# ysong1231/SimRank

Hardware: AMD Instinct MI355X
Metric: simrank_iterations_per_sec (higher is better)
Workload: dtype f32

## Files before the change

simrank_amd/csrc/api.hip:

```cpp
#include <algorithm>
#include <chrono>
#include <cstring>
#include <mutex>
#include <unordered_map>
#include <string>
#include <thread>
#include <vector>

#include "common.h"

namespace simrank {

static thread_local char g_err[512] = "";

void set_error(const char* fmt, ...) {
    va_list ap;
    va_start(ap, fmt);
    vsnprintf(g_err, sizeof(g_err), fmt, ap);
    va_end(ap);
}

Tuning& tuning() {
    static Tuning t;
    return t;
// ... 884 lines not shown
    } else if (!strcmp(key, "fuse_sym")) {
        SR_REQUIRE(value >= -1 && value <= 1, "fuse_sym must be -1 (automatic), 0 or 1");
        t.fuse_sym = value;
    } else if (!strcmp(key, "fuse_steps")) {
        SR_REQUIRE(value >= -1 && value <= (1 << 20), "fuse_steps must be >= 0, or -1 (by the operand's size)");
        t.fuse_steps = value;
    } else if (!strcmp(key, "fuse_dens")) {
        SR_REQUIRE(value >= 0 && value <= (1 << 20), "fuse_dens must be >= 0");
        t.fuse_dens = value;
    } else if (!strcmp(key, "dense_cols")) {
        SR_REQUIRE(value >= 1 && value <= (1 << 20), "dense_cols must be >= 1");
        t.dense_cols = value;
    } else if (!strcmp(key, "restrict_support")) {
        SR_REQUIRE(value >= -1 && value <= 1, "restrict_support must be -1 (automatic), 0 or 1");
        t.restrict_support = value;
    } else {
        SR_REQUIRE(false, "unknown tuning key '%s'", key);
    }
    return SIMRANK_OK;
}

int simrank_get_tuning(const char* key, int64_t* value) {
    SR_REQUIRE(key && value, "NULL argument");
    const Tuning t = tuning_snapshot();
    if (!strcmp(key, "panel")) *value = t.panel;
    else if (!strcmp(key, "xcd_map")) *value = t.xcd_map;
    else if (!strcmp(key, "stream_nt")) *value = t.stream_nt;
    else if (!strcmp(key, "tile")) *value = t.tile;
    else if (!strcmp(key, "triangle")) *value = t.triangle;
    else if (!strcmp(key, "huge")) *value = t.huge;
// ... 15 lines not shown
    else if (!strcmp(key, "ev_tri")) *value = t.ev_tri;
    else if (!strcmp(key, "fuse_rows")) *value = t.fuse_rows;
    else if (!strcmp(key, "fuse_wgs")) *value = t.fuse_wgs;
    else if (!strcmp(key, "fuse_max_rows")) *value = t.fuse_max_rows;
    else if (!strcmp(key, "fuse_order")) *value = t.fuse_order;
    else if (!strcmp(key, "fuse_store")) *value = t.fuse_store;
    else if (!strcmp(key, "fuse_meta_nt")) *value = t.fuse_meta_nt;
    else if (!strcmp(key, "sym_desc")) *value = t.sym_desc;
    else if (!strcmp(key, "ids16")) *value = t.ids16;
    else if (!strcmp(key, "lean")) *value = t.lean;
    else if (!strcmp(key, "addr32")) *value = t.addr32;
    else if (!strcmp(key, "probe_flags")) *value = t.probe_flags;
    else if (!strcmp(key, "dense_terms")) *value = t.dense_terms;
    else if (!strcmp(key, "probe_mask")) *value = t.probe_mask;
    else if (!strcmp(key, "restrict_support")) *value = t.restrict_support;
    else SR_REQUIRE(false, "unknown tuning key '%s'", key);
    return SIMRANK_OK;
}

int simrank_graph_get(const simrank_graph* g, const char* key, int64_t* value) {
    SR_REQUIRE(g && key && value, "NULL argument");
    if (!strcmp(key, "fused_ids16")) *value = g->fused ? g->fused->ids16 : -1;
    else if (!strcmp(key, "gather_ids16")) *value = (g->col16 && g->tun.ids16) ? 1 : 0;
    else SR_REQUIRE(false, "unknown graph key '%s'", key);
    return SIMRANK_OK;
}

}
```

simrank_amd/csrc/common.h:

```cpp
#pragma once
#include <hip/hip_runtime.h>

#include <cstdarg>
#include <atomic>
#include <cstdint>
#include <cstdio>
#include <cstdlib>
#include <cstring>
#include <functional>
#include <vector>

#include "simrank_hip.h"

namespace simrank {

void set_error(const char* fmt, ...);

#define SR_HIP(call)                                                                   \
    do {                                                                               \
        hipError_t e_ = (call);                                                        \
        if (e_ != hipSuccess) {                                                        \
            ::simrank::set_error("%s failed: %s (%s:%d)", #call, hipGetErrorString(e_), \
                                 __FILE__, __LINE__);                                  \
            return SIMRANK_ERR_HIP;                                                    \
// ... 31 lines not shown
    int64_t fuse_min = 0;
    int64_t fuse_pays = -1;
    int64_t fuse_steps = -1;
    int64_t fuse_dens = 0;
    int64_t fuse_unit = 48;
    int64_t fuse_rows = 8192;
    int64_t fuse_store = 1;
    int64_t fuse_meta_nt = 0;
    int64_t fuse_order = 0;
    int64_t fuse_max_rows = 1 << 20;
    int64_t fuse_cap = 40000;
    int64_t fuse_wgs = 4;
    int64_t fuse_shards = 1;
    int64_t fuse_group = 3;
    int64_t fuse_sym = -1;
    int64_t dense_lazy = 0;
    int64_t dense_sym = -1;
    int64_t restrict_support = -1;
};
inline int32_t restrict_choice(const Tuning& t, int64_t live, int64_t total) {
    return t.restrict_support < 0 ? (2 * live < total ? 1 : 0) : int32_t(t.restrict_support != 0);
}
Tuning& tuning();
Tuning tuning_snapshot();


#ifdef SIMRANK_HOST_ONLY
inline hipError_t plan_alloc(void** p, size_t bytes) {
    *p = malloc(bytes ? bytes : 1);
    return *p ? hipSuccess : hipErrorOutOfMemory;
// ... 25 lines not shown
int rows_to_host(const void* S, int64_t rows_pad, int64_t n, const int32_t* inv_dev, const int32_t* rows, int32_t n_rows,
                 float* dst, int64_t ld, int elem, float scale, hipStream_t stream);
inline hipError_t pool_hip_alloc(void** p, size_t bytes) {
    const int rc = pool_alloc(p, bytes);
    return rc == SIMRANK_OK ? hipSuccess : (rc == SIMRANK_ERR_ALLOC ? hipErrorOutOfMemory : hipErrorUnknown);
}

int identity_leg1_blocked(const simrank_graph* g, float* Tt, int64_t t_rows_pad, void* stream);
int identity_leg1_blocked_h16(const simrank_graph* g, uint16_t* Tt, int64_t t_rows_pad, float scale, void* stream);

struct PlanPrep {
    std::vector<int32_t> ord, inv;
    std::vector<int32_t> rp, cl;
    std::vector<float> rs;
    bool asym = false;
};
struct BiPlanPrep {
    std::vector<int32_t> rowptr21, col21;
    std::vector<int32_t> ord[2], inv[2];
    std::vector<int32_t> rp[2], cl[2];
    std::vector<float> rs[2];
    bool asym = false;
};
int plan_prepare(int64_t n, int64_t nnz, const int32_t* rowptr, const int32_t* col, const float* rowscale,
                 const simrank_plan_options* opt, PlanPrep* out);
int shard_prepare(int64_t n, int64_t nnz, const int32_t* rowptr, const int32_t* col, const float* rowscale,
                  const float* apriori, int64_t ld_apriori, bool reorder, int32_t deal, PlanPrep* out, bool allow_asym = false);
int shard_biplan_prepare(int64_t n1, int64_t n2, int64_t nnz, const int32_t* rowptr12, const int32_t* col12,
                         const float* rowscale1, const float* rowscale2, const simrank_biplan_options* opt, int32_t deal1,
                         int32_t deal2, BiPlanPrep* out, bool allow_asym = false);
bool prior_symmetric(const float* a, int64_t ld, int64_t n);
// ... 45 lines not shown
    int64_t n_quads = 0;
    int64_t n_steps = 0;
    int64_t nnz_covered = 0;
    int64_t r_nnz = 0;
    int32_t* units = nullptr;
    int32_t n_pslots = 0, n_cslots = 0;
    float* partials = nullptr;
    int32_t* tickets = nullptr;
    int32_t cap_panels = 0;
    uint16_t* dcols16 = nullptr;
    int32_t* dcols32 = nullptr;
    uint4* abits = nullptr;
    int2* gmeta = nullptr;
    uint16_t* sids16 = nullptr;
    int32_t* sids32 = nullptr;
};

#ifdef SIMRANK_EXPERIMENT_FUSED2
struct simrank_fused2_plan {
    int32_t n_items = 0;
    int32_t n_blocks = 0;
    int32_t ids16 = 0;
    int32_t cap_panels = 0;
    int64_t n_quads = 0, n_steps = 0, nnz_covered = 0, r_nnz = 0;
    int32_t* items = nullptr;
    int32_t n_pslots = 0, n_cslots = 0;
    float* partials = nullptr;
    int32_t* tickets = nullptr;
    uint32_t* heads = nullptr;
    uint16_t* dcols16 = nullptr;
    int32_t* dcols32 = nullptr;
    uint4* abits = nullptr;
    int2* gmeta = nullptr;
    uint16_t* sids16 = nullptr;
    int32_t* sids32 = nullptr;
};
#endif

namespace simrank {
constexpr int kFB = 128;
constexpr int kSub = 4;
void free_fused_plan(simrank_fused_plan* p);
int build_fused_plan(simrank_graph* g, const int32_t* rowptr, const int32_t* col, const float* rowscale);
int launch_fused_trans(const simrank_graph* g, const float* X, int64_t x_rows_pad, int64_t L, float* Y,
                       int64_t y_rows_pad, hipStream_t st);
bool fused_sym_applies(const simrank_graph* g, int64_t x_rows_pad, int64_t L, int64_t y_rows_pad);
int launch_fused_sym(const simrank_graph* g, const float* X, int64_t x_rows_pad, int64_t L, float* Y, int64_t y_rows_pad,
                     float coef, float lbd, double eps, const uint8_t* ev, const float* ap, const float* prev,
                     unsigned long long* n_changed, int32_t set_diag, int32_t count_any, hipStream_t st);
bool fused_rowmajor_fits(const simrank_graph* g, const float* X, int64_t ldx, int64_t L, const float* Y, int64_t t_block,
                         int64_t t_pad);
int launch_fused_trans_rowmajor(const simrank_graph* g, const float* X, int64_t ldx, int64_t L, float* Y, int64_t t_block,
                                int64_t t_pad, hipStream_t st);
#ifdef SIMRANK_EXPERIMENT_FUSED2
void free_fused2_plan(simrank_fused2_plan* p);
int build_fused2_plan(simrank_graph* g, const int32_t* rowptr, const int32_t* col, const float* rowscale);
int launch_fused2_trans(const simrank_graph* g, const float* X, int64_t x_rows_pad, int64_t L, float* Y,
                        int64_t y_rows_pad, hipStream_t st);
#endif
struct DenseUse {
// ... 40 lines not shown
```

simrank_amd/csrc/fused.hip:

```cpp
#include <algorithm>
#include <cstring>
#include <numeric>
#include <vector>

#include <cstdlib>

#include <mutex>
#include <thread>

#include "common.h"
#include "fused_dev.h"

namespace simrank {

constexpr int kTS = 132;
#ifndef SIMRANK_KMINUNITS
#define SIMRANK_KMINUNITS 64
#endif
#ifndef SIMRANK_KGROUPENTRIES
#define SIMRANK_KGROUPENTRIES 6144
#endif
#ifndef SIMRANK_KMAXREM
#define SIMRANK_KMAXREM 256
#endif
// ... 23 lines not shown
    int32_t* tickets;
    int32_t n_pslots, n_cslots;
    const uint16_t* dcols16;
    const int32_t* dcols32;
    const uint4* abits;
    const int2* gmeta;
    const uint16_t* sids16;
    const int32_t* sids32;
    float coef, lbd;
    double eps;
    const uint8_t* ev;
    const float* ap;
    const float* prev;
    unsigned long long* n_changed;
    int32_t set_diag, count_any;
};

#ifndef SIMRANK_HOST_ONLY
#if defined(__HIP_DEVICE_COMPILE__) && !defined(__gfx942__) && !defined(__gfx950__)
#error "fused.hip: the sc1 hand-off between the units of a split block is written for gfx942 / gfx950"
#endif
#ifdef SIMRANK_FUSED_STAMPS
constexpr int kFstCap = 1 << 15;
__device__ unsigned long long g_fst[kFstCap * 8];
__device__ unsigned int g_fst_base;
__device__ __forceinline__ unsigned long long fst_now() {
    unsigned long long t;
    __builtin_amdgcn_sched_barrier(0);
    asm volatile("s_memtime %0\n\ts_waitcnt lgkmcnt(0)" : "=s"(t) :: "memory");
    __builtin_amdgcn_sched_barrier(0);
// ... 32 lines not shown
    const int32_t* un = p.units + size_t(unit) * 32;
    FST(0);
#ifdef SIMRANK_FUSED_STAMPS
    if (threadIdx.x == 0 && blockIdx.x - g_fst_base < unsigned(kFstCap)) {
        const unsigned xcc = __builtin_amdgcn_s_getreg((4 - 1) << 11 | 0 << 6 | 20);
        const unsigned hw = __builtin_amdgcn_s_getreg((16 - 1) << 11 | 0 << 6 | 4);
        g_fst[size_t(blockIdx.x - g_fst_base) * 8 + 5] = (unsigned long long)xcc << 32 | hw;
        g_fst[size_t(blockIdx.x - g_fst_base) * 8 + 6] = (unsigned long long)panel << 32 | unit;
    }
#endif
    const int b0 = un[0];
    const int64_t c0 = int64_t(panel) * 32;
    const int n_sub_all = un[8];
    const int n_sub_sym = SYM ? min(n_sub_all, int((c0 + 31) >> 7) - b0 + 1) : n_sub_all;
    if (SYM && n_sub_sym <= 0) return;
    const int g = lane >> 3, q = lane & 7, gbase = lane & ~7;
    const uint32_t qoff = uint32_t(q) * 16u;

    const float* xbase = p.X + int64_t(panel) * p.x_panel_stride;
    const __amdgpu_buffer_rsrc_t srd = __builtin_amdgcn_make_buffer_rsrc(
        const_cast<float*>(xbase), 0, p.x_bytes - (p.x_pitch == 128u ? 0 : panel * 128), 0x00020000);
    const uint32_t pitch = p.x_pitch;
    const int sent = p.x_sentinel;

    const int quad0 = un[1];
    const int nq = (p.probe & 4) ? 0 : un[2];
    const int unit_k = un[3], unit_nb = un[4], pslot = un[5], cslot = un[6];
    const bool has_set = !(p.probe & 4) && un[7] != 0;
    const int n_sub = n_sub_sym;
    const int per = (nq + 3) >> 2;
// ... 832 lines not shown
            std::fwrite(sids.data(), sizeof(int32_t), sids.size(), f);
            std::fwrite(dcols.data(), sizeof(int32_t), dcols.size(), f);
            std::fclose(f);
        }
    }
    simrank_fused_plan* pl = new simrank_fused_plan;
    pl->n_units = (int32_t)(units.size() / 32);
    pl->n_blocks = (int32_t)nblk;
    pl->n_pslots = n_pslots;
    pl->n_cslots = n_cslots;
    pl->n_quads = blk_quad0[size_t(nblk)];
    pl->n_steps = steps_total;
    pl->nnz_covered = covered;
    pl->r_nnz = r_nnz;
    pl->ids16 = ids16 ? 1 : 0;
    dcols.resize(dcols.size() + 64, 0);
    abits.resize(abits.size() + 64 * 4, 0u);
    int rc = upload_vec(&pl->units, units);
    if (!rc) {
        if (ids16) {
            std::vector<uint16_t> d16(dcols.begin(), dcols.end());
            rc = upload_vec(&pl->dcols16, d16);
        } else {
            rc = upload_vec(&pl->dcols32, dcols);
        }
    }
    if (!rc) rc = upload_vec(reinterpret_cast<uint32_t**>(&pl->abits), abits);
    if (!rc) rc = upload_vec(reinterpret_cast<int32_t**>(&pl->gmeta), blk_gmeta);
    if (!rc) {
        if (ids16) {
// ... 73 lines not shown
        if (pl->ids16)
            hipLaunchKernelGGL((fused_trans_kernel<true, true>), dim3((unsigned)grid), dim3(256), lds_pad, st, a);
        else
            hipLaunchKernelGGL((fused_trans_kernel<false, true>), dim3((unsigned)grid), dim3(256), lds_pad, st, a);
    } else if (pl->ids16) {
        hipLaunchKernelGGL((fused_trans_kernel<true, false>), dim3((unsigned)grid), dim3(256), lds_pad, st, a);
    } else {
        hipLaunchKernelGGL((fused_trans_kernel<false, false>), dim3((unsigned)grid), dim3(256), lds_pad, st, a);
    }
#endif
    SR_HIP(hipGetLastError());
    return SIMRANK_OK;
}

int launch_fused_trans(const simrank_graph* g, const float* X, int64_t x_rows_pad, int64_t L, float* Y,
                       int64_t y_rows_pad, hipStream_t st) {
    SR_REQUIRE(g->fused, "graph has no fused plan");
    SR_REQUIRE(aligned16(X) && aligned16(Y), "fused leg needs 16-byte aligned operands");
    SR_REQUIRE(x_rows_pad >= g->n_cols && (x_rows_pad + 1) * 128 < (int64_t(1) << 31) && x_rows_pad < (int64_t(1) << 24) - 1,
               "fused leg: operand of %lld rows per panel", (long long)x_rows_pad);
    FusedArgs a{};
    a.X = X; a.Y = Y;
    a.x_rows_pad = x_rows_pad; a.y_rows_pad = y_rows_pad;
    a.L = L;
    a.x_panel_stride = x_rows_pad * 32;
    a.x_pitch = 128;
    a.x_bytes = int32_t(x_rows_pad * 128);
    a.x_sentinel = (int32_t)x_rows_pad;
    return launch_fused(g, a, st);
}

bool fused_sym_applies(const simrank_graph* g, int64_t x_rows_pad, int64_t L, int64_t y_rows_pad) {
    const simrank_fused_plan* pl = g->fused;
    if (!pl || !g->tun.fuse || g->tun.fuse_sym == 0 || g->tun.dense_terms != 3) return false;
    if (L != g->n_rows || g->n_cols > g->tun.fuse_max_rows) return false;
    if ((x_rows_pad + 1) * 128 >= (int64_t(1) << 31) || (y_rows_pad + 1) * 128 >= (int64_t(1) << 31) ||
        x_rows_pad >= (int64_t(1) << 24) - 1 || y_rows_pad >= (int64_t(1) << 24) - 1)
        return false;
    if (g->tun.fuse_sym < 0) return 2 * pl->nnz_covered >= g->nnz;
    return true;
}

int launch_fused_sym(const simrank_graph* g, const float* X, int64_t x_rows_pad, int64_t L, float* Y, int64_t y_rows_pad,
                     float coef, float lbd, double eps, const uint8_t* ev, const float* ap, const float* prev,
// ... 72 lines not shown
```

simrank_amd/csrc/plan.hip:

```cpp
#include <algorithm>
#include <chrono>
#include <cstdlib>
#include <cstring>
#include <numeric>
#include <vector>

#include "loop.h"
#include "side.h"

struct simrank_plan {
    simrank::side_t s;
    unsigned long long* counters = nullptr;
    unsigned long long* host_counters[2] = {nullptr, nullptr};
    hipEvent_t counted[2] = {nullptr, nullptr};
    hipStream_t stream = nullptr;
    int32_t asym = 0;
    int32_t updates = 0;
    int32_t identity_leg1 = 1;
    int32_t at_identity = 0;
    std::vector<hipEvent_t> ev_pool;
    std::vector<hipEvent_t> ev_used;
    bool timing = false;
};

// ... 103 lines not shown
    }
    if (p->s.half && !p->s.g->fused) {
        set_error("storage_fp16 needs the one-launch plan (tuning fuse = 1) and a graph that has one");
        return fail(SIMRANK_ERR_INVALID);
    }
    auto counters = [&]() -> int {
        SIDE_HIP(pool_hip_alloc((void**)&p->counters, sizeof(unsigned long long) * SIMRANK_CHANGED_SLOTS));
        for (int i = 0; i < 2; ++i) {
            SIDE_HIP(hipHostMalloc((void**)&p->host_counters[i], sizeof(unsigned long long) * SIMRANK_CHANGED_SLOTS, hipHostMallocPortable));
            SIDE_HIP(hipEventCreateWithFlags(&p->counted[i], hipEventDisableTiming));
        }
        return SIMRANK_OK;
    };
    rc = counters();
    if (!rc) rc = side_alloc(a, pp.ord, pp.inv, p->stream);
    if (rc) return fail(rc);
    lap("matrices allocated, orders uploaded, stream drained");
    if (opt->evidence) rc = side_restrict(a, p->stream);
    if (!rc && opt->apriori) rc = side_prior(a, opt->apriori, opt->ld_apriori, p->stream);
    if (rc) return fail(rc);
    lap("live segments, prior");
    rc = simrank_plan_reset(p);
    if (rc) return fail(rc);
    lap("reset queued");
    *out = p;
    return SIMRANK_OK;
}

int simrank_plan_reset(simrank_plan* p) {
    SR_REQUIRE(p, "plan is NULL");
// ... 149 lines not shown
```

simrank_amd/csrc/planprep.hip:

```cpp
#include <algorithm>
#include <atomic>
#include <cmath>
#include <numeric>
#include <thread>

#include "common.h"

namespace simrank {

static int check_csr(int64_t n_rows, int64_t n_cols, int64_t nnz, const int32_t* rowptr, const int32_t* col) {
    SR_REQUIRE(rowptr[0] == 0 && rowptr[n_rows] == nnz, "rowptr does not span [0, nnz]");
    for (int64_t a = 0; a < n_rows; ++a)
        SR_REQUIRE(rowptr[a + 1] >= rowptr[a] && rowptr[a + 1] <= nnz, "rowptr not monotone at row %lld", (long long)a);
    for (int64_t j = 0; j < nnz; ++j) SR_REQUIRE(col[j] >= 0 && col[j] < n_cols, "column index %d out of range", col[j]);
    return SIMRANK_OK;
}

static int check_prior(const float* a, int64_t ld, int64_t n, int which, bool half, bool* asym = nullptr) {
    if (!a) return SIMRANK_OK;
    SR_REQUIRE(ld >= n, "prior %d: ld %lld < n", which, (long long)ld);
    for (int64_t i = 0; i < n; ++i)
        for (int64_t j = i; j < n; ++j) {
            const float v = a[i * ld + j];
            if (j > i && !(v == a[j * ld + i])) {
// ... 61 lines not shown
    }
    SR_REQUIRE(dup_row.load() < 0, "duplicate entry in row %d%s", ord[(size_t)dup_row.load()], what);
    return SIMRANK_OK;
}

static void length_order(int64_t n, const int32_t* rowptr, bool reorder, std::vector<int32_t>& ord, std::vector<int32_t>& inv) {
    ord.resize((size_t)n);
    inv.resize((size_t)n);
    std::iota(ord.begin(), ord.end(), 0);
    if (reorder)
        std::stable_sort(ord.begin(), ord.end(),
                         [rowptr](int32_t x, int32_t y) { return rowptr[x + 1] - rowptr[x] < rowptr[y + 1] - rowptr[y]; });
    for (int64_t r = 0; r < n; ++r) inv[(size_t)ord[(size_t)r]] = (int32_t)r;
}

static void deal_order(int64_t n, int32_t deal, std::vector<int32_t>& ord, std::vector<int32_t>& inv) {
    if (deal <= 1 || n % (32 * int64_t(deal))) return;
    const int64_t unit = n % (128 * int64_t(deal)) == 0 ? 128 : 32, per = n / (unit * deal);
    std::vector<int32_t> dealt((size_t)n);
    for (int64_t b = 0; b < per; ++b)
        for (int64_t w = 0; w < deal; ++w)
            for (int64_t i = 0; i < unit; ++i)
                dealt[(size_t)((w * per + b) * unit + i)] = ord[(size_t)((b * deal + w) * unit + i)];
    ord.swap(dealt);
    for (int64_t r = 0; r < n; ++r) inv[(size_t)ord[(size_t)r]] = (int32_t)r;
}

int plan_prepare(int64_t n, int64_t nnz, const int32_t* rowptr, const int32_t* col, const float* rowscale,
                 const simrank_plan_options* opt, PlanPrep* out) {
    SR_REQUIRE(opt && rowptr && rowscale && (col || nnz == 0) && n > 0 && nnz >= 0 && out, "bad plan arguments");
    SR_REQUIRE(n < (int64_t(1) << 24) - 16, "a plan holds at most 2^24 nodes");
    SR_REQUIRE(opt->dense_terms == 0 || opt->dense_terms == 1 || opt->dense_terms == 3, "dense_terms must be 0, 1 or 3");
    int rc = check_csr(n, n, nnz, rowptr, col);
    out->asym = false;
    if (!rc) rc = check_prior(opt->apriori, opt->ld_apriori, n, 1, opt->storage_fp16 != 0, &out->asym);
    if (rc) return rc;
    length_order(n, rowptr, opt->reorder != 0, out->ord, out->inv);
    return renamed(n, rowptr, col, rowscale, out->ord, out->inv, nnz, "", out->rp, out->cl, out->rs);
}

int shard_prepare(int64_t n, int64_t nnz, const int32_t* rowptr, const int32_t* col, const float* rowscale,
                  const float* apriori, int64_t ld_apriori, bool reorder, int32_t deal, PlanPrep* out, bool allow_asym) {
    SR_REQUIRE(rowptr && rowscale && (col || nnz == 0) && n > 0 && nnz >= 0 && out, "bad plan arguments");
    SR_REQUIRE(n < (int64_t(1) << 24) - 16, "a plan holds at most 2^24 nodes");
    int rc = check_csr(n, n, nnz, rowptr, col);
    out->asym = false;
    if (!rc) rc = check_prior(apriori, ld_apriori, n, 1, false, allow_asym ? &out->asym : nullptr);
    if (rc) return rc;
    length_order(n, rowptr, reorder, out->ord, out->inv);
    if (reorder) deal_order(n, deal, out->ord, out->inv);
    return renamed(n, rowptr, col, rowscale, out->ord, out->inv, nnz, "", out->rp, out->cl, out->rs);
}

// ... 75 lines not shown
```

simrank_amd/csrc/side.h:

```cpp
#pragma once
#include <cstring>
#include <vector>

#include "common.h"

namespace simrank {

constexpr float kHalfScale = 16384.0f;

#define SIDE_HIP(call)                                                                            \
    do {                                                                                          \
        hipError_t e_ = (call);                                                                   \
        if (e_ != hipSuccess) {                                                                   \
            set_error("%s failed: %s (%s:%d)", #call, hipGetErrorString(e_), __FILE__, __LINE__); \
            (void)hipGetLastError();                                                              \
            return e_ == hipErrorOutOfMemory ? SIMRANK_ERR_ALLOC : SIMRANK_ERR_HIP;               \
        }                                                                                         \
    } while (0)

struct side_t {
    int64_t n = 0, k = 0, rows_pad = 0, k_rows_pad = 0;
    size_t mat_bytes = 0, t_bytes = 0;
    simrank_graph* g = nullptr;
    float* S[2] = {nullptr, nullptr};
    float* Tt = nullptr;
    uint8_t* ev = nullptr;
    float* prior = nullptr;
    int32_t* inv = nullptr;
    int32_t* ord_dev = nullptr;
    std::vector<int32_t> ord;
    float coef = 0.8f, lbd = 0.f;
    int32_t restrict_support = 0;
    int32_t half = 0;
    int cur = 0;
};

inline size_t side_f32_bytes(const side_t& a) { return size_t((a.n + 31) / 32) * size_t(a.rows_pad) * 32 * sizeof(float); }

inline void side_shape(side_t& a, int64_t n, int64_t k, bool half) {
    a.n = n;
    a.k = k;
    a.half = half ? 1 : 0;
    a.rows_pad = (n + 7) / 8 * 8 + 8;
    a.k_rows_pad = (k + 7) / 8 * 8 + 8;
    const size_t panels = half ? size_t((n + 63) / 64) : size_t((n + 31) / 32);
    a.mat_bytes = panels * size_t(a.rows_pad) * 128;
    a.t_bytes = panels * size_t(a.k_rows_pad) * 128;
}

// ... 5 lines not shown
    SIDE_HIP(hipMemcpyAsync(a.inv, inv.data(), ids, hipMemcpyHostToDevice, st));
    a.ord = ord;
    SIDE_HIP(pool_hip_alloc((void**)&a.ord_dev, ids));
    SIDE_HIP(hipMemcpyAsync(a.ord_dev, a.ord.data(), ids, hipMemcpyHostToDevice, st));
    SIDE_HIP(hipStreamSynchronize(st));
    return SIMRANK_OK;
}

inline void side_trim(side_t& a) {
    (void)pool_free(a.S[0]); (void)pool_free(a.S[1]); (void)pool_free(a.Tt); (void)pool_free(a.prior);
    a.S[0] = a.S[1] = a.Tt = a.prior = nullptr;
}

inline void side_free(side_t& a) {
    side_trim(a);
    (void)pool_free(a.ev); (void)pool_free(a.inv); (void)pool_free(a.ord_dev);
    simrank_graph_destroy(a.g);
}

inline int side_reset(side_t& a, hipStream_t st) {
    a.cur = 0;
    if (a.half) return simrank_fill_identity_blocked_h16(a.S[0], a.n, a.n, a.rows_pad, 0, kHalfScale, st);
    return simrank_fill_identity_blocked(a.S[0], a.n, a.n, a.rows_pad, 0, st);
}

inline int side_evidence_alloc(side_t& a, int fill, hipStream_t st) {
    const size_t ev_bytes = size_t((a.n + 31) / 32) * size_t(a.rows_pad) * 32;
    hipError_t e = pool_hip_alloc((void**)&a.ev, ev_bytes);
    if (e == hipSuccess) e = hipMemsetAsync(a.ev, fill, ev_bytes, st);
    if (e != hipSuccess) {
        set_error("evidence counts: %s", hipGetErrorString(e));
// ... 24 lines not shown
        rc = simrank_permute_layout(tmp, n, 0, a.prior, 32, a.rows_pad, n, n, a.ord_dev, a.ord_dev, 4, st);
        e = hipStreamSynchronize(st);
    }
    (void)pool_free(tmp);
    if (e != hipSuccess) {
        set_error("plan prior upload: %s", hipGetErrorString(e));
        return SIMRANK_ERR_HIP;
    }
    return rc;
}

template <class Stamp>
int side_leg_pair(side_t& a, const side_t& o, bool from_identity, bool asym, double eps, int32_t exact_count,
                  unsigned long long* counters, unsigned long long* host_slot, hipStream_t st, Stamp&& stamp) {
    const int nx = a.cur ^ 1;
    int rc = stamp();
    if (rc) return rc;
    rc = from_identity ? (a.half ? identity_leg1_blocked_h16(a.g, reinterpret_cast<uint16_t*>(a.Tt), a.k_rows_pad, kHalfScale, st)
                                 : identity_leg1_blocked(a.g, a.Tt, a.k_rows_pad, st))
         : a.half ? simrank_spmm_blocked_h16(a.g, o.S[o.cur], o.rows_pad, a.k, a.Tt, a.k_rows_pad, 1, nullptr, 0, kHalfScale, st)
                  : simrank_spmm_blocked(a.g, o.S[o.cur], o.rows_pad, a.k, a.Tt, a.k_rows_pad, 1, nullptr, st);
    if (!rc) rc = stamp();
    if (rc) return rc;
    simrank_epilogue ep{};
    ep.coef = a.coef;
    ep.lbd = a.lbd;
    ep.evidence = a.ev;
    ep.ld_evidence = 32;
    ep.apriori = a.prior;
    ep.ld_apriori = 32;
    ep.previous = a.S[a.cur];
    ep.ld_previous = 32;
    ep.eps = eps;
    ep.n_changed = counters;
    ep.diag_col0 = 0;
    ep.set_diag = 1;
    ep.symmetric = 1;
    ep.restrict_support = a.restrict_support;
    ep.count_any = exact_count ? 0 : 1;
    if (asym) {
        ep.symmetric = 0;
        ep.restrict_support = 0;
        rc = simrank_spmm_blocked(a.g, a.Tt, a.k_rows_pad, a.n, a.S[nx], a.rows_pad, 1, nullptr, st);
        if (!rc) rc = simrank_epilogue_apply_blocked(a.S[nx], a.S[nx], a.n, a.n, a.rows_pad, &ep, st);
    } else {
        rc = a.half ? simrank_spmm_blocked_h16(a.g, a.Tt, a.k_rows_pad, a.n, a.S[nx], a.rows_pad, 0, &ep, a.rows_pad, kHalfScale, st)
                    : simrank_spmm_blocked(a.g, a.Tt, a.k_rows_pad, a.n, a.S[nx], a.rows_pad, 0, &ep, st);
    }
    if (!rc) rc = stamp();
    if (rc) return rc;
    SR_HIP(hipMemcpyAsync(host_slot, counters, sizeof(unsigned long long) * SIMRANK_CHANGED_SLOTS, hipMemcpyDeviceToHost, st));
    return SIMRANK_OK;
}

// ... 74 lines not shown
        const int64_t node = a.ord[(size_t)r];
        std::memcpy(idx_host + node * k, idx_s.data() + r * k, size_t(k) * sizeof(int32_t));
        std::memcpy(val_host + node * k, val_s.data() + r * k, size_t(k) * sizeof(float));
    }
    return SIMRANK_OK;
}

inline int side_get(const side_t& a, const char* key, int64_t* value) {
    if (!strcmp(key, "restrict_support")) *value = a.restrict_support;
    else if (!strcmp(key, "iterate")) *value = (int64_t)(uintptr_t)a.S[a.cur];
    else if (!strcmp(key, "iterate_layout")) *value = a.half ? 2 : 0;
    else if (!strcmp(key, "iterate_stride")) *value = a.rows_pad;
    else if (!strcmp(key, "iterate_rows") || !strcmp(key, "iterate_col_hi")) *value = a.n;
    else if (!strcmp(key, "iterate_col_lo")) *value = 0;
    else if (!strcmp(key, "ids")) *value = (int64_t)(uintptr_t)a.ord_dev;
    else SR_REQUIRE(false, "unknown plan key '%s'", key);
    return SIMRANK_OK;
}

}
```

simrank_amd/csrc/spmm.hip:

```cpp
#include <algorithm>
#include <type_traits>

#include <mutex>

#include "common.h"

namespace simrank {

__device__ __forceinline__ int64_t imin(int64_t a, int64_t b) { return a < b ? a : b; }

__device__ __forceinline__ int64_t elem_at(int64_t r, int64_t c, int64_t ld, int64_t rows_pad) {
    return rows_pad ? ((c >> 5) * rows_pad + r) * 32 + (c & 31) : r * ld + c;
}

struct SpmmArgs {
    const int32_t* rowptr;
    const int32_t* col;
    const uint16_t* col16;
    int32_t blocked;
    int64_t x_rows_pad, y_rows_pad;
    int64_t x_span_bytes;
    int32_t x_sentinel;
    int32_t addr32;
    int32_t sh_rank, sh_mb;
// ... 1772 lines not shown
    *total = n_rows * ((n_cols + 31) / 32);
    return SIMRANK_OK;
}

int simrank_fill_identity(float* S, int64_t n_rows, int64_t n_cols, int64_t ld, int64_t col0,
                          void* stream) {
    SR_REQUIRE(S && n_rows > 0 && n_cols > 0 && ld >= n_cols, "bad identity block");
    const int64_t total = n_rows * n_cols;
    const int grid = (int)std::min<int64_t>((total + 255) / 256, 256 * 16);
    hipLaunchKernelGGL(fill_identity_kernel, dim3(grid), dim3(256), 0, as_stream(stream), S,
                       n_rows, n_cols, ld, col0);
    SR_HIP(hipGetLastError());
    return SIMRANK_OK;
}

static int spmm_impl(const simrank_graph* g, const float* X, int64_t ldx, int64_t n_cols_x,
                     float* Y, int64_t ldy, int32_t transpose_out, int64_t t_block, int64_t t_pad,
                     const simrank_epilogue* ep, void* stream, bool blocked, int64_t x_rows_pad,
                     int64_t y_rows_pad) {
    SR_REQUIRE(t_pad >= 0 && t_pad < 4096, "t_pad out of range");
    SR_REQUIRE(g && X && Y, "NULL argument");
    const Tuning& T = g->tun;
    SR_REQUIRE(!(transpose_out && ep), "an epilogue needs transpose_out = 0");
    SpmmArgs a{};
    a.blocked = blocked ? 1 : 0;
    a.x_rows_pad = x_rows_pad;
    a.y_rows_pad = y_rows_pad;
    a.rowptr = g->rowptr;
    a.col = g->col;
    a.col16 = T.ids16 ? g->col16 : nullptr;
    a.rowscale = g->rowscale;
    a.huge_len = (int32_t)std::max<int64_t>(kHeavy, T.huge);
    a.has_huge = g->max_row_nnz >= a.huge_len ? 1 : 0;
    a.X = X;
// ... 27 lines not shown
        a.ld_prev = ep->ld_previous;
        a.eps = ep->eps;
        a.n_changed = ep->n_changed;
        a.diag_col0 = ep->diag_col0;
        a.set_diag = ep->set_diag;
        a.restrict_support = ep->restrict_support;
        a.count_any = ep->count_any;
        if (blocked) a.ld_ev = a.ld_ap = a.ld_prev = 32;
        SR_REQUIRE(!a.ev || a.ld_ev >= n_cols_x || blocked, "evidence ld too small");
        SR_REQUIRE(!a.ap || a.ld_ap >= n_cols_x || blocked, "apriori ld too small");
        SR_REQUIRE(!a.prev || ((a.ld_prev >= n_cols_x || blocked) && a.n_changed),
                   "previous needs ld >= columns and a counter");
        if (a.ev) vec_ok = vec_ok && (reinterpret_cast<uintptr_t>(a.ev) % 4 == 0) && a.ld_ev % 4 == 0;
        if (a.ap) vec_ok = vec_ok && aligned16(a.ap) && a.ld_ap % 4 == 0;
        if (a.prev) vec_ok = vec_ok && aligned16(a.prev) && a.ld_prev % 4 == 0;
        if (a.prev) SR_HIP(hipMemsetAsync(a.n_changed, 0, sizeof(unsigned long long) * SIMRANK_CHANGED_SLOTS, st));
    }
    int64_t panel = T.panel;
    if (panel == 0) panel = transpose_out ? 32 : 64;
    int64_t tile = T.tile;
    if (tile == 0) tile = 32;
    a.nt = (int32_t)T.stream_nt;
    const bool want_sym = ep && ep->symmetric && T.triangle && vec_ok && !transpose_out &&
                          n_cols_x == g->n_rows && ep->diag_col0 == 0 && g->n_rows >= 64;
    if (blocked && transpose_out && g->fused && T.fuse && vec_ok && T.dense_terms == 3 && g->n_cols <= T.fuse_max_rows &&
        (x_rows_pad + 1) * 128 < (int64_t(1) << 31)) {
#ifdef SIMRANK_EXPERIMENT_FUSED2
        if (T.fuse == 2 && g->fused2 && (g->fused2->n_pslots == 0 || (n_cols_x + 31) / 32 <= g->fused2->cap_panels))
            return launch_fused2_trans(g, X, x_rows_pad, n_cols_x, Y, y_rows_pad, st);
#endif
        return launch_fused_trans(g, X, x_rows_pad, n_cols_x, Y, y_rows_pad, st);
    }
    if (!blocked && transpose_out && g->fused && T.fuse && T.fuse_shards && vec_ok && T.dense_terms == 3 &&
        g->n_cols <= T.fuse_max_rows) {
        const int64_t tb = a.tstride ? g->n_rows : t_block, tp = a.tstride ? a.tstride - g->n_rows : t_pad;
        if (fused_rowmajor_fits(g, X, ldx, n_cols_x, Y, tb, tp))
            return launch_fused_trans_rowmajor(g, X, ldx, n_cols_x, Y, tb, tp, st);
    }
    if (blocked && want_sym && !transpose_out && ep && (!ep->restrict_support || T.fuse_sym > 0) &&
        fused_sym_applies(g, x_rows_pad, n_cols_x, y_rows_pad))
        return launch_fused_sym(g, X, x_rows_pad, n_cols_x, Y, y_rows_pad, a.coef, a.lbd, a.eps, a.ev, a.ap, a.prev, a.n_changed,
                                a.set_diag, a.count_any, st);
    const simrank_dense_plan* dp = (vec_ok && T.dense_min > 0 && tile == 32) ? g->dense : nullptr;
    if (dp && want_sym) {
        const int64_t mode = T.dense_sym;
        if (mode == 0 || (mode < 0 && 2 * dp->nnz_covered < g->nnz)) dp = nullptr;
    }
    if (dp) {
        DenseUse use;
        const int rc = launch_dense_tiles(g, X, blocked ? -x_rows_pad : ldx, n_cols_x, want_sym, st, &use);
        if (rc) return rc;
        a.dpart = use.part;
        a.ldp = use.ldp;
        a.dslab0 = use.block_slab0;
        a.dnslab = use.block_nslab;
        a.rowptr = dp->r_rowptr;
        a.col = dp->r_col;
        a.col16 = T.ids16 ? dp->r_col16 : nullptr;
        a.has_huge = dp->r_max_row >= a.huge_len ? 1 : 0;
    }
    if (T.balance) {
        const int32_t* tr0 = dp ? dp->r_tile_row0 : g->tile_row0;
// ... 141 lines not shown
    SR_REQUIRE(n_cols_x > 0 && ldx >= n_cols_x, "X: %lld columns, ld %lld", (long long)n_cols_x,
               (long long)ldx);
    SR_REQUIRE(transpose_out || ldy >= n_cols_x, "Y: ld %lld < %lld columns", (long long)ldy,
               (long long)n_cols_x);
    return spmm_impl(g, X, ldx, n_cols_x, Y, ldy, transpose_out, t_block, t_pad, ep, stream, false, 0, 0);
}

int simrank_spmm_blocked(const simrank_graph* g, const float* X, int64_t x_rows_pad, int64_t n_cols_x,
                         float* Y, int64_t y_rows_pad, int32_t transpose_out,
                         const simrank_epilogue* ep, void* stream) {
    SR_REQUIRE(g && n_cols_x > 0, "bad arguments");
    SR_REQUIRE(x_rows_pad >= g->n_cols && y_rows_pad >= (transpose_out ? n_cols_x : g->n_rows),
               "padded row counts %lld / %lld too small", (long long)x_rows_pad, (long long)y_rows_pad);
    return spmm_impl(g, X, 32, n_cols_x, Y, 32, transpose_out, 0, 0, ep, stream, true, x_rows_pad, y_rows_pad);
}

static int epilogue_apply_impl(const float* Q, int64_t ldq, float* Y, int64_t ldy, int64_t n_rows,
                               int64_t n_cols, const simrank_epilogue* ep, void* stream, int64_t rows_pad) {
    SR_REQUIRE(Q && Y && ep, "NULL argument");
    SR_REQUIRE(n_rows > 0 && n_cols > 0 && (rows_pad ? rows_pad >= n_rows : (ldq >= n_cols && ldy >= n_cols)),
               "bad block shape");
    SpmmArgs a{};
    a.y_rows_pad = rows_pad;
    a.has_ep = 1;
    a.coef = ep->coef;
    a.lbd = ep->lbd;
    a.ev = ep->evidence;
    a.ld_ev = ep->ld_evidence;
    a.ap = ep->apriori;
    a.ld_ap = ep->ld_apriori;
// ... 300 lines not shown
```

Baseline: 134.7.

## Skip leg-1 fused work units whose output the triangular second leg never reads

Builds a per-panel first-referenced-block table on the host and passes it to the fused transposed SpMM kernel. Work units whose last block falls before the first block the triangular symmetric second leg will read exit early. A refined node ordering (by length, then first reference) is added to concentrate skippable work. A dry-run of the spmm dispatcher checks that the second leg really is triangular before skipping is enabled. The cost is extra host preprocessing, a device table, and reliance on the triangle path only reading the upper part.

```diff
diff --git a/simrank_amd/csrc/api.hip b/simrank_amd/csrc/api.hip
--- a/simrank_amd/csrc/api.hip
+++ b/simrank_amd/csrc/api.hip
@@ -922,6 +922,11 @@
     } else if (!strcmp(key, "restrict_support")) {
         SR_REQUIRE(value >= -1 && value <= 1, "restrict_support must be -1 (automatic), 0 or 1");
         t.restrict_support = value;
+    } else if (!strcmp(key, "leg1_skip")) {
+        t.leg1_skip = value ? 1 : 0;
+    } else if (!strcmp(key, "leg1_order")) {
+        SR_REQUIRE(value >= -1 && value <= 1, "leg1_order must be -1 (by the graph's size), 0 or 1");
+        t.leg1_order = value;
     } else {
         SR_REQUIRE(false, "unknown tuning key '%s'", key);
     }
@@ -967,6 +972,8 @@
     else if (!strcmp(key, "dense_terms")) *value = t.dense_terms;
     else if (!strcmp(key, "probe_mask")) *value = t.probe_mask;
     else if (!strcmp(key, "restrict_support")) *value = t.restrict_support;
+    else if (!strcmp(key, "leg1_skip")) *value = t.leg1_skip;
+    else if (!strcmp(key, "leg1_order")) *value = t.leg1_order;
     else SR_REQUIRE(false, "unknown tuning key '%s'", key);
     return SIMRANK_OK;
 }
diff --git a/simrank_amd/csrc/common.h b/simrank_amd/csrc/common.h
--- a/simrank_amd/csrc/common.h
+++ b/simrank_amd/csrc/common.h
@@ -69,6 +69,8 @@
     int64_t fuse_shards = 1;
     int64_t fuse_group = 3;
     int64_t fuse_sym = -1;
+    int64_t leg1_skip = 1;
+    int64_t leg1_order = -1;
     int64_t dense_lazy = 0;
     int64_t dense_sym = -1;
     int64_t restrict_support = -1;
@@ -124,7 +126,10 @@
     std::vector<int32_t> rp, cl;
     std::vector<float> rs;
     bool asym = false;
-};
+    std::vector<int32_t> first_block;
+};
+constexpr int32_t kLeg1Never = 0x7FFFFFFF;
+void first_block_table(int64_t n, const int32_t* rp, const int32_t* cl, std::vector<int32_t>& first_block);
 struct BiPlanPrep {
     std::vector<int32_t> rowptr21, col21;
     std::vector<int32_t> ord[2], inv[2];
@@ -200,6 +205,7 @@
     int2* gmeta = nullptr;
     uint16_t* sids16 = nullptr;
     int32_t* sids32 = nullptr;
+    std::vector<int32_t> unit_last;
 };
 
 #ifdef SIMRANK_EXPERIMENT_FUSED2
@@ -229,7 +235,12 @@
 void free_fused_plan(simrank_fused_plan* p);
 int build_fused_plan(simrank_graph* g, const int32_t* rowptr, const int32_t* col, const float* rowscale);
 int launch_fused_trans(const simrank_graph* g, const float* X, int64_t x_rows_pad, int64_t L, float* Y,
-                       int64_t y_rows_pad, hipStream_t st);
+                       int64_t y_rows_pad, hipStream_t st, const int32_t* first_block = nullptr);
+void fused_leg1_counts(const simrank_graph* g, int64_t L, const int32_t* first_block_host, int64_t* units, int64_t* skipped);
+int spmm_blocked_is_triangle(const simrank_graph* g, const float* X, int64_t x_rows_pad, int64_t n_cols_x, float* Y,
+                             int64_t y_rows_pad, const simrank_epilogue* ep, bool* triangle);
+int spmm_blocked_leg1(const simrank_graph* g, const float* X, int64_t x_rows_pad, int64_t n_cols_x, float* Y,
+                      int64_t y_rows_pad, const int32_t* first_block, bool* skipping, void* stream);
 bool fused_sym_applies(const simrank_graph* g, int64_t x_rows_pad, int64_t L, int64_t y_rows_pad);
 int launch_fused_sym(const simrank_graph* g, const float* X, int64_t x_rows_pad, int64_t L, float* Y, int64_t y_rows_pad,
                      float coef, float lbd, double eps, const uint8_t* ev, const float* ap, const float* prev,
diff --git a/simrank_amd/csrc/fused.hip b/simrank_amd/csrc/fused.hip
--- a/simrank_amd/csrc/fused.hip
+++ b/simrank_amd/csrc/fused.hip
@@ -61,6 +61,7 @@
     const float* prev;
     unsigned long long* n_changed;
     int32_t set_diag, count_any;
+    const int32_t* first_block;
 };
 
 #ifndef SIMRANK_HOST_ONLY
@@ -123,6 +124,9 @@
     const int n_sub_all = un[8];
     const int n_sub_sym = SYM ? min(n_sub_all, int((c0 + 31) >> 7) - b0 + 1) : n_sub_all;
     if (SYM && n_sub_sym <= 0) return;
+    if constexpr (!SYM) {
+        if (p.first_block && b0 + n_sub_all - 1 < p.first_block[panel]) return;
+    }
     const int g = lane >> 3, q = lane & 7, gbase = lane & ~7;
     const uint32_t qoff = uint32_t(q) * 16u;
 
@@ -985,6 +989,9 @@
     pl->nnz_covered = covered;
     pl->r_nnz = r_nnz;
     pl->ids16 = ids16 ? 1 : 0;
+    pl->unit_last.reserve(ulist.size());
+    for (const Unit& u : ulist) pl->unit_last.push_back(u.b0 + u.nsub - 1);
+    std::sort(pl->unit_last.begin(), pl->unit_last.end());
     dcols.resize(dcols.size() + 64, 0);
     abits.resize(abits.size() + 64 * 4, 0u);
     int rc = upload_vec(&pl->units, units);
@@ -1088,7 +1095,7 @@
 }
 
 int launch_fused_trans(const simrank_graph* g, const float* X, int64_t x_rows_pad, int64_t L, float* Y,
-                       int64_t y_rows_pad, hipStream_t st) {
+                       int64_t y_rows_pad, hipStream_t st, const int32_t* first_block) {
     SR_REQUIRE(g->fused, "graph has no fused plan");
     SR_REQUIRE(aligned16(X) && aligned16(Y), "fused leg needs 16-byte aligned operands");
     SR_REQUIRE(x_rows_pad >= g->n_cols && (x_rows_pad + 1) * 128 < (int64_t(1) << 31) && x_rows_pad < (int64_t(1) << 24) - 1,
@@ -1101,7 +1108,19 @@
     a.x_pitch = 128;
     a.x_bytes = int32_t(x_rows_pad * 128);
     a.x_sentinel = (int32_t)x_rows_pad;
+    a.first_block = first_block;
     return launch_fused(g, a, st);
+}
+
+void fused_leg1_counts(const simrank_graph* g, int64_t L, const int32_t* first_block_host, int64_t* units, int64_t* skipped) {
+    *units = *skipped = 0;
+    const simrank_fused_plan* pl = g->fused;
+    if (!pl) return;
+    const int64_t n_panels = (L + 31) / 32;
+    *units = n_panels * pl->n_units;
+    if (!first_block_host) return;
+    for (int64_t p = 0; p < n_panels; ++p)
+        *skipped += std::lower_bound(pl->unit_last.begin(), pl->unit_last.end(), first_block_host[p]) - pl->unit_last.begin();
 }
 
 bool fused_sym_applies(const simrank_graph* g, int64_t x_rows_pad, int64_t L, int64_t y_rows_pad) {
diff --git a/simrank_amd/csrc/plan.hip b/simrank_amd/csrc/plan.hip
--- a/simrank_amd/csrc/plan.hip
+++ b/simrank_amd/csrc/plan.hip
@@ -141,6 +141,17 @@
     };
     rc = counters();
     if (!rc) rc = side_alloc(a, pp.ord, pp.inv, p->stream);
+    if (!rc && !a.half) {
+        auto table = [&]() -> int {
+            const size_t bytes = pp.first_block.size() * sizeof(int32_t);
+            SIDE_HIP(pool_hip_alloc((void**)&a.first_block, bytes));
+            SIDE_HIP(hipMemcpyAsync(a.first_block, pp.first_block.data(), bytes, hipMemcpyHostToDevice, p->stream));
+            SIDE_HIP(hipStreamSynchronize(p->stream));
+            a.first_block_host = pp.first_block;
+            return SIMRANK_OK;
+        };
+        rc = table();
+    }
     if (rc) return fail(rc);
     lap("matrices allocated, orders uploaded, stream drained");
     if (opt->evidence) rc = side_restrict(a, p->stream);
diff --git a/simrank_amd/csrc/planprep.hip b/simrank_amd/csrc/planprep.hip
--- a/simrank_amd/csrc/planprep.hip
+++ b/simrank_amd/csrc/planprep.hip
@@ -99,6 +99,35 @@
     for (int64_t r = 0; r < n; ++r) inv[(size_t)ord[(size_t)r]] = (int32_t)r;
 }
 
+static void refine_by_first_reference(int64_t n, const int32_t* rowptr, const int32_t* col, std::vector<int32_t>& ord,
+                                      std::vector<int32_t>& inv) {
+    std::vector<int32_t> first((size_t)n);
+    for (int pass = 0; pass < 2; ++pass) {
+        std::fill(first.begin(), first.end(), (int32_t)n);
+        for (int64_t r = 0; r < n; ++r) {
+            const int32_t a = ord[(size_t)r];
+            for (int32_t j = rowptr[a]; j < rowptr[a + 1]; ++j)
+                if (first[(size_t)col[j]] == (int32_t)n) first[(size_t)col[j]] = (int32_t)r;
+        }
+        std::stable_sort(ord.begin(), ord.end(), [&](int32_t x, int32_t y) {
+            const int32_t lx = rowptr[x + 1] - rowptr[x], ly = rowptr[y + 1] - rowptr[y];
+            return lx != ly ? lx < ly : first[(size_t)x] < first[(size_t)y];
+        });
+    }
+    for (int64_t r = 0; r < n; ++r) inv[(size_t)ord[(size_t)r]] = (int32_t)r;
+}
+
+void first_block_table(int64_t n, const int32_t* rp, const int32_t* cl, std::vector<int32_t>& first_block) {
+    std::vector<int32_t> first((size_t)n, kLeg1Never);
+    for (int64_t a = 0; a < n; ++a)
+        for (int32_t j = rp[a]; j < rp[a + 1]; ++j)
+            if (first[(size_t)cl[j]] == kLeg1Never) first[(size_t)cl[j]] = (int32_t)a;
+    first_block.assign((size_t)((n + 31) / 32), kLeg1Never);
+    for (int64_t i = 0; i < n; ++i)
+        if (first[(size_t)i] != kLeg1Never)
+            first_block[(size_t)(i >> 5)] = std::min(first_block[(size_t)(i >> 5)], first[(size_t)i] / 128);
+}
+
 static void deal_order(int64_t n, int32_t deal, std::vector<int32_t>& ord, std::vector<int32_t>& inv) {
     if (deal <= 1 || n % (32 * int64_t(deal))) return;
     const int64_t unit = n % (128 * int64_t(deal)) == 0 ? 128 : 32, per = n / (unit * deal);
@@ -121,7 +150,13 @@
     if (!rc) rc = check_prior(opt->apriori, opt->ld_apriori, n, 1, opt->storage_fp16 != 0, &out->asym);
     if (rc) return rc;
     length_order(n, rowptr, opt->reorder != 0, out->ord, out->inv);
-    return renamed(n, rowptr, col, rowscale, out->ord, out->inv, nnz, "", out->rp, out->cl, out->rs);
+    const Tuning t = tuning_snapshot();
+    const bool refine = t.leg1_order > 0 || (t.leg1_order < 0 && n >= kSpeculateBelow);
+    if (opt->reorder && refine && t.triangle && t.fuse == 1 && n >= 64 && !out->asym && !opt->storage_fp16)
+        refine_by_first_reference(n, rowptr, col, out->ord, out->inv);
+    rc = renamed(n, rowptr, col, rowscale, out->ord, out->inv, nnz, "", out->rp, out->cl, out->rs);
+    if (!rc) first_block_table(n, out->rp.data(), out->cl.data(), out->first_block);
+    return rc;
 }
 
 int shard_prepare(int64_t n, int64_t nnz, const int32_t* rowptr, const int32_t* col, const float* rowscale,
diff --git a/simrank_amd/csrc/side.h b/simrank_amd/csrc/side.h
--- a/simrank_amd/csrc/side.h
+++ b/simrank_amd/csrc/side.h
@@ -33,6 +33,10 @@
     int32_t restrict_support = 0;
     int32_t half = 0;
     int cur = 0;
+    int32_t* first_block = nullptr;
+    std::vector<int32_t> first_block_host;
+    int64_t leg1_units = 0, leg1_skipped = 0;
+    int64_t dead_units = -1;
 };
 
 inline size_t side_f32_bytes(const side_t& a) { return size_t((a.n + 31) / 32) * size_t(a.rows_pad) * 32 * sizeof(float); }
@@ -68,7 +72,7 @@
 
 inline void side_free(side_t& a) {
     side_trim(a);
-    (void)pool_free(a.ev); (void)pool_free(a.inv); (void)pool_free(a.ord_dev);
+    (void)pool_free(a.ev); (void)pool_free(a.inv); (void)pool_free(a.ord_dev); (void)pool_free(a.first_block);
     simrank_graph_destroy(a.g);
 }
 
@@ -123,14 +127,6 @@
 int side_leg_pair(side_t& a, const side_t& o, bool from_identity, bool asym, double eps, int32_t exact_count,
                   unsigned long long* counters, unsigned long long* host_slot, hipStream_t st, Stamp&& stamp) {
     const int nx = a.cur ^ 1;
-    int rc = stamp();
-    if (rc) return rc;
-    rc = from_identity ? (a.half ? identity_leg1_blocked_h16(a.g, reinterpret_cast<uint16_t*>(a.Tt), a.k_rows_pad, kHalfScale, st)
-                                 : identity_leg1_blocked(a.g, a.Tt, a.k_rows_pad, st))
-         : a.half ? simrank_spmm_blocked_h16(a.g, o.S[o.cur], o.rows_pad, a.k, a.Tt, a.k_rows_pad, 1, nullptr, 0, kHalfScale, st)
-                  : simrank_spmm_blocked(a.g, o.S[o.cur], o.rows_pad, a.k, a.Tt, a.k_rows_pad, 1, nullptr, st);
-    if (!rc) rc = stamp();
-    if (rc) return rc;
     simrank_epilogue ep{};
     ep.coef = a.coef;
     ep.lbd = a.lbd;
@@ -147,6 +143,31 @@
     ep.symmetric = 1;
     ep.restrict_support = a.restrict_support;
     ep.count_any = exact_count ? 0 : 1;
+    const int32_t* skip = nullptr;
+    if (a.first_block && a.g->tun.leg1_skip && !from_identity && !asym && !a.half) {
+        bool triangle = false;
+        const int rct = spmm_blocked_is_triangle(a.g, a.Tt, a.k_rows_pad, a.n, a.S[nx], a.rows_pad, &ep, &triangle);
+        if (rct) return rct;
+        if (triangle) skip = a.first_block;
+    }
+    int rc = stamp();
+    if (rc) return rc;
+    bool skipping = false;
+    rc = from_identity ? (a.half ? identity_leg1_blocked_h16(a.g, reinterpret_cast<uint16_t*>(a.Tt), a.k_rows_pad, kHalfScale, st)
+                                 : identity_leg1_blocked(a.g, a.Tt, a.k_rows_pad, st))
+         : a.half ? simrank_spmm_blocked_h16(a.g, o.S[o.cur], o.rows_pad, a.k, a.Tt, a.k_rows_pad, 1, nullptr, 0, kHalfScale, st)
+                  : spmm_blocked_leg1(a.g, o.S[o.cur], o.rows_pad, a.k, a.Tt, a.k_rows_pad, skip, &skipping, st);
+    a.leg1_units = a.leg1_skipped = 0;
+    if (!rc && a.first_block && !from_identity && !a.half) {
+        int64_t dead = 0;
+        fused_leg1_counts(a.g, a.k, skipping ? a.first_block_host.data() : nullptr, &a.leg1_units, &dead);
+        if (skipping) {
+            if (a.dead_units < 0) a.dead_units = dead;
+            a.leg1_skipped = a.dead_units;
+        }
+    }
+    if (!rc) rc = stamp();
+    if (rc) return rc;
     if (asym) {
         ep.symmetric = 0;
         ep.restrict_support = 0;
@@ -251,6 +272,8 @@
     else if (!strcmp(key, "iterate_rows") || !strcmp(key, "iterate_col_hi")) *value = a.n;
     else if (!strcmp(key, "iterate_col_lo")) *value = 0;
     else if (!strcmp(key, "ids")) *value = (int64_t)(uintptr_t)a.ord_dev;
+    else if (!strcmp(key, "leg1_units")) *value = a.leg1_units;
+    else if (!strcmp(key, "leg1_skipped")) *value = a.leg1_skipped;
     else SR_REQUIRE(false, "unknown plan key '%s'", key);
     return SIMRANK_OK;
 }
diff --git a/simrank_amd/csrc/spmm.hip b/simrank_amd/csrc/spmm.hip
--- a/simrank_amd/csrc/spmm.hip
+++ b/simrank_amd/csrc/spmm.hip
@@ -1810,10 +1810,15 @@
     return SIMRANK_OK;
 }
 
+struct Leg1Skip {
+    bool dry = false, triangle = false, skipping = false;
+    const int32_t* first_block = nullptr;
+};
+
 static int spmm_impl(const simrank_graph* g, const float* X, int64_t ldx, int64_t n_cols_x,
                      float* Y, int64_t ldy, int32_t transpose_out, int64_t t_block, int64_t t_pad,
                      const simrank_epilogue* ep, void* stream, bool blocked, int64_t x_rows_pad,
-                     int64_t y_rows_pad) {
+                     int64_t y_rows_pad, Leg1Skip* sk = nullptr) {
     SR_REQUIRE(t_pad >= 0 && t_pad < 4096, "t_pad out of range");
     SR_REQUIRE(g && X && Y, "NULL argument");
     const Tuning& T = g->tun;
@@ -1871,7 +1876,8 @@
         if (a.ev) vec_ok = vec_ok && (reinterpret_cast<uintptr_t>(a.ev) % 4 == 0) && a.ld_ev % 4 == 0;
         if (a.ap) vec_ok = vec_ok && aligned16(a.ap) && a.ld_ap % 4 == 0;
         if (a.prev) vec_ok = vec_ok && aligned16(a.prev) && a.ld_prev % 4 == 0;
-        if (a.prev) SR_HIP(hipMemsetAsync(a.n_changed, 0, sizeof(unsigned long long) * SIMRANK_CHANGED_SLOTS, st));
+        if (a.prev && !(sk && sk->dry))
+            SR_HIP(hipMemsetAsync(a.n_changed, 0, sizeof(unsigned long long) * SIMRANK_CHANGED_SLOTS, st));
     }
     int64_t panel = T.panel;
     if (panel == 0) panel = transpose_out ? 32 : 64;
@@ -1880,13 +1886,25 @@
     a.nt = (int32_t)T.stream_nt;
     const bool want_sym = ep && ep->symmetric && T.triangle && vec_ok && !transpose_out &&
                           n_cols_x == g->n_rows && ep->diag_col0 == 0 && g->n_rows >= 64;
+    const bool one_launch_sym = blocked && want_sym && !transpose_out && ep && (!ep->restrict_support || T.fuse_sym > 0) &&
+                                fused_sym_applies(g, x_rows_pad, n_cols_x, y_rows_pad);
+    const simrank_dense_plan* dp = (vec_ok && T.dense_min > 0 && tile == 32) ? g->dense : nullptr;
+    if (dp && want_sym) {
+        const int64_t mode = T.dense_sym;
+        if (mode == 0 || (mode < 0 && 2 * dp->nnz_covered < g->nnz)) dp = nullptr;
+    }
+    if (sk && sk->dry) {
+        sk->triangle = blocked && want_sym && (one_launch_sym || !dp);
+        return SIMRANK_OK;
+    }
     if (blocked && transpose_out && g->fused && T.fuse && vec_ok && T.dense_terms == 3 && g->n_cols <= T.fuse_max_rows &&
         (x_rows_pad + 1) * 128 < (int64_t(1) << 31)) {
 #ifdef SIMRANK_EXPERIMENT_FUSED2
         if (T.fuse == 2 && g->fused2 && (g->fused2->n_pslots == 0 || (n_cols_x + 31) / 32 <= g->fused2->cap_panels))
             return launch_fused2_trans(g, X, x_rows_pad, n_cols_x, Y, y_rows_pad, st);
 #endif
-        return launch_fused_trans(g, X, x_rows_pad, n_cols_x, Y, y_rows_pad, st);
+        if (sk) sk->skipping = sk->first_block != nullptr;
+        return launch_fused_trans(g, X, x_rows_pad, n_cols_x, Y, y_rows_pad, st, sk ? sk->first_block : nullptr);
     }
     if (!blocked && transpose_out && g->fused && T.fuse && T.fuse_shards && vec_ok && T.dense_terms == 3 &&
         g->n_cols <= T.fuse_max_rows) {
@@ -1894,15 +1912,9 @@
         if (fused_rowmajor_fits(g, X, ldx, n_cols_x, Y, tb, tp))
             return launch_fused_trans_rowmajor(g, X, ldx, n_cols_x, Y, tb, tp, st);
     }
-    if (blocked && want_sym && !transpose_out && ep && (!ep->restrict_support || T.fuse_sym > 0) &&
-        fused_sym_applies(g, x_rows_pad, n_cols_x, y_rows_pad))
+    if (one_launch_sym)
         return launch_fused_sym(g, X, x_rows_pad, n_cols_x, Y, y_rows_pad, a.coef, a.lbd, a.eps, a.ev, a.ap, a.prev, a.n_changed,
                                 a.set_diag, a.count_any, st);
-    const simrank_dense_plan* dp = (vec_ok && T.dense_min > 0 && tile == 32) ? g->dense : nullptr;
-    if (dp && want_sym) {
-        const int64_t mode = T.dense_sym;
-        if (mode == 0 || (mode < 0 && 2 * dp->nnz_covered < g->nnz)) dp = nullptr;
-    }
     if (dp) {
         DenseUse use;
         const int rc = launch_dense_tiles(g, X, blocked ? -x_rows_pad : ldx, n_cols_x, want_sym, st, &use);
@@ -2074,6 +2086,30 @@
                "padded row counts %lld / %lld too small", (long long)x_rows_pad, (long long)y_rows_pad);
     return spmm_impl(g, X, 32, n_cols_x, Y, 32, transpose_out, 0, 0, ep, stream, true, x_rows_pad, y_rows_pad);
 }
+
+}
+
+namespace simrank {
+int spmm_blocked_is_triangle(const simrank_graph* g, const float* X, int64_t x_rows_pad, int64_t n_cols_x, float* Y,
+                             int64_t y_rows_pad, const simrank_epilogue* ep, bool* triangle) {
+    Leg1Skip sk;
+    sk.dry = true;
+    const int rc = spmm_impl(g, X, 32, n_cols_x, Y, 32, 0, 0, 0, ep, nullptr, true, x_rows_pad, y_rows_pad, &sk);
+    *triangle = rc == SIMRANK_OK && sk.triangle;
+    return rc;
+}
+
+int spmm_blocked_leg1(const simrank_graph* g, const float* X, int64_t x_rows_pad, int64_t n_cols_x, float* Y,
+                      int64_t y_rows_pad, const int32_t* first_block, bool* skipping, void* stream) {
+    Leg1Skip sk;
+    sk.first_block = first_block;
+    const int rc = spmm_impl(g, X, 32, n_cols_x, Y, 32, 1, 0, 0, nullptr, stream, true, x_rows_pad, y_rows_pad, &sk);
+    *skipping = rc == SIMRANK_OK && sk.skipping;
+    return rc;
+}
+}
+
+extern "C" {
 
 static int epilogue_apply_impl(const float* Q, int64_t ldq, float* Y, int64_t ldy, int64_t n_rows,
                                int64_t n_cols, const simrank_epilogue* ep, void* stream, int64_t rows_pad) {
```

New measurement: 142.8 (median of 6 runs). 6.0% higher.
